# wangrui2025/GDKVM

Hardware: AMD Instinct MI355X
Metric: frames/sec (GDKVM forward + argmax mask), EchoNet 112x112x32 clips (higher is better)
Workload: dtype bf16; 1 GPU; BASELINE.json configs[1]: EchoNet-Dynamic 112x112x32 bf16 inference, batch=16 per GPU; clips_per_gpu=16, frames_per_clip=32, image=112x112, heads=1, key_dim=64, rule=delta_sequential, world_size=1, ranks_seen=1

## Files before the change

gdkvm_amd/csrc/conv3x3_tile.hip:

```cpp
#include <atomic>
#include "gdkvm_device.hpp"

namespace {

constexpr int CT_CK = 64;
constexpr int CT_PIX = 160;
constexpr int CT_SLOTS = CT_PIX / 16;
constexpr int CT_MAXMT = 13;
constexpr int CT_VARIANT_128 = 4, CT_VARIANT_64 = 3;

struct ConvTileArgs {
    const bf16_t* x; const bf16_t* w; const float* bias; const bf16_t* res; bf16_t* y;
    const bf16_t* x2; int C1;
    int N, H, W, C, K;
    int fpt, th, tiles_y, ntiles;
    int bw, bh, band_px, npieces;
    int relu;
    float inv_band, inv_bw, inv_tw, inv_w;
    int perm;
};

__host__ __device__ __forceinline__ int ct_channel(int kt, int j, int perm)
{
    return perm ? 32 * (kt >> 1) + 8 * (j >> 2) + 4 * (kt & 1) + (j & 3) : 16 * kt + j;
}

template <int NWN, int NTW, bool PK, int NWV = 8, int MAXMT = CT_MAXMT>
__global__ __launch_bounds__(64 * NWV, (NWV == 4 ? 2 : 1)) void conv3x3_tile_kernel(ConvTileArgs a)
{
    constexpr int MW = NWV / NWN, MTW = (MAXMT + MW - 1) / MW;
    extern __shared__ __attribute__((aligned(16))) unsigned char ct_band[];
    const int tid = threadIdx.x, lane = tid & 63, li = lane & 15, g = lane >> 4;
    const int w = __builtin_amdgcn_readfirstlane(tid >> 6), wn = w % NWN, wm = w / NWN;
    const int H = a.H, W = a.W, C = a.C, K = a.K, BW = a.bw;
    const int band_bytes = a.npieces * 1024, nchunk = C / CT_CK;
    const int tpix = a.fpt * a.th * W;
    const int co0 = blockIdx.y * (16 * NTW * NWN) + 16 * NTW * wn;

    f32x4 bias4[NTW];
#pragma unroll
    for (int nt = 0; nt < NTW; ++nt) {
        const int kt = min(co0 / 16 + nt, K / 16 - 1);
        const float* bp = a.bias + ct_channel(kt, 4 * g, a.perm);
        asm volatile("global_load_dwordx4 %0, %1, off" : "=&v"(bias4[nt]) : "v"(bp) : "memory");
    }

    constexpr int PP = NWV == 8 ? 7 : 8;
    const int cs1 = a.C1, cs2 = a.x2 ? C - a.C1 : C;
    unsigned g_off1[PP], g_off2[PP];
#pragma unroll
    for (int u = 0; u < PP; ++u) {
        const int j = w + NWV * u, d = 64 * j + lane, pix = d / CT_SLOTS, c = d - CT_SLOTS * pix;
        const int f = idx_div(pix, a.inv_band), r = pix - f * (a.bh * BW), by = idx_div(r, a.inv_bw), bx = r - by * BW;
        const int sp = (f * H + by - 1) * W + bx - 1;
        const bool live = j < a.npieces && c < 8 && pix < a.band_px && bx >= 1 && bx <= W && (a.tiles_y > 1 || (by >= 1 && by <= a.th));
        g_off1[u] = live ? (unsigned)(sp * cs1 * 2 + c * 16) : RSRC_DEAD;
        g_off2[u] = live ? (unsigned)(sp * cs2 * 2 + c * 16) : RSRC_DEAD;
    }
    const unsigned lds0 = (unsigned)reinterpret_cast<uintptr_t>(ct_band);
    const int nlive = max(0, (a.npieces - w + NWV - 1) / NWV);
    struct Geo { int px0, npx, row0; };
    auto geo_of = [&](int tile) __attribute__((always_inline)) {
        const int ty = tile % a.tiles_y, fg = tile / a.tiles_y;
        Geo q;
        q.px0 = fg * a.fpt * H * W;
        q.npx = min(a.fpt, a.N - fg * a.fpt) * H * W;
        q.row0 = ty * a.th * W;
        return q;
    };
    auto fetch = [&](const Geo q, int chunk, int buf) __attribute__((always_inline)) {
        const bool second = a.x2 != nullptr && chunk * CT_CK >= a.C1;
        const int cs = second ? cs2 : cs1;
        const bf16_t* base = (second ? a.x2 : a.x) + (long long)q.px0 * cs;
        const __amdgpu_buffer_rsrc_t rsrc = make_rsrc(base, q.npx * cs * 2);
        const unsigned ts = (unsigned)((q.row0 * cs + chunk * CT_CK - (second ? a.C1 : 0)) * 2);
        const unsigned dst0 = lds0 + buf * band_bytes + 1024 * w;
#pragma unroll
        for (int u = 0; u < PP; ++u) {
            const unsigned dst = u < nlive ? dst0 + 1024 * NWV * u : lds0 + 2 * band_bytes;
            __builtin_amdgcn_raw_ptr_buffer_load_lds(rsrc, lds_dma_dst(dst), 16,
                                                     (int)((second ? g_off2[u] : g_off1[u]) + ts), 0, 0, 0);
        }
    };

    int tile = blockIdx.x;
    Geo cur = geo_of(min(tile, a.ntiles - 1));
    if (tile < a.ntiles) fetch(cur, 0, 0);

    unsigned pbase[MTW];
#pragma unroll
    for (int m = 0; m < MTW; ++m) {
        const int p = min(16 * (wm + MW * m) + li, tpix - 1);
        const int f = idx_div(p, a.inv_tw), r = p - f * (a.th * W), py = idx_div(r, a.inv_w), px = r - py * W;
        pbase[m] = (unsigned)(((f * a.bh + py) * BW + px) * CT_PIX + g * 16);
    }
    const bf16_t* wrow[NTW];
#pragma unroll
    for (int nt = 0; nt < NTW; ++nt) {
        const int kt = min(co0 / 16 + nt, K / 16 - 1);
        if constexpr (PK) wrow[nt] = a.w + (size_t)kt * (9 * C * 16) + lane * 8;
        else wrow[nt] = a.w + (size_t)ct_channel(kt, li, a.perm) * 9 * C + 8 * g;
    }

    const int nks = nchunk * 18;
    static_assert(NTW == 1 || NTW == 2, "wwait names the fragments of one or two output tiles");
    struct WF { bf16x8 f[NTW]; };
    auto wload = [&](WF& o, int ks) __attribute__((always_inline)) {
        ks = ks >= nks ? ks - nks : ks;
        size_t off;
        if constexpr (PK) off = (size_t)ks * 512;
        else {
            const int chunk = ks / 18, r = ks - 18 * chunk, tap = r >> 1, kh = r & 1;
            off = (size_t)tap * C + chunk * CT_CK + 32 * kh;
        }
#pragma unroll
        for (int nt = 0; nt < NTW; ++nt) asm volatile("global_load_dwordx4 %0, %1, off" : "=&v"(o.f[nt]) : "v"(wrow[nt] + off) : "memory");
    };
    auto wwait = [&](WF& o, auto nc) __attribute__((always_inline)) {
        constexpr int N = decltype(nc)::value;
        if constexpr (NTW == 1) asm volatile("s_waitcnt vmcnt(%1)" : "+v"(o.f[0]) : "n"(N) : "memory");
        else asm volatile("s_waitcnt vmcnt(%2)" : "+v"(o.f[0]), "+v"(o.f[1]) : "n"(N) : "memory");
    };
    int gc = 0;
    constexpr int WD = 3, KU = 6;
    WF wr[WD];
#pragma unroll
    for (int j = 0; j < WD; ++j) wload(wr[j], j);
    for (; tile < a.ntiles; tile += gridDim.x) {
        const Geo nxt = geo_of(min(tile + (int)gridDim.x, a.ntiles - 1));
        f32x4 acc[MTW][NTW];
#pragma unroll
        for (int m = 0; m < MTW; ++m)
#pragma unroll
            for (int nt = 0; nt < NTW; ++nt) acc[m][nt] = f32x4{0.f, 0.f, 0.f, 0.f};
        for (int chunk = 0; chunk < nchunk; ++chunk, ++gc) {
            const int buf = gc & 1;
            asm volatile("s_waitcnt vmcnt(%0) lgkmcnt(0)" ::"n"(WD * NTW) : "memory");
            asm volatile("s_barrier" ::: "memory");
            {
                const bool more = chunk + 1 < nchunk;
                Geo q;
                q.px0 = more ? cur.px0 : nxt.px0; q.npx = more ? cur.npx : nxt.npx; q.row0 = more ? cur.row0 : nxt.row0;
                fetch(q, more ? chunk + 1 : 0, buf ^ 1);
            }
            const unsigned char* band = ct_band + buf * band_bytes;
            auto load_x = [&](bf16x8 (&xb)[MTW], int r) __attribute__((always_inline)) {
                r = min(r, 17);
                const int tap = r >> 1, kh = r & 1, dy = tap / 3, dx = tap - 3 * dy;
                const unsigned off = (unsigned)((dy * BW + dx) * CT_PIX + kh * 64);
#pragma unroll
                for (int m = 0; m < MTW; ++m) {
                    xb[m] = *reinterpret_cast<const bf16x8*>(band + pbase[m] + off);
                }
            };
            auto mfmas = [&](const bf16x8 (&xb)[MTW], const WF& wfr) __attribute__((always_inline)) {
#pragma unroll
                for (int m = 0; m < MTW; ++m)
#pragma unroll
                    for (int nt = 0; nt < NTW; ++nt) {
                        acc[m][nt] = __builtin_amdgcn_mfma_f32_16x16x32_bf16(wfr.f[nt], xb[m], acc[m][nt], 0, 0, 0);
                    }
            };
            const int ksb = chunk * 18;
            bf16x8 xa[MTW], xb[MTW];
            load_x(xa, 0);
            auto trip = [&](int r0, auto firstc) __attribute__((always_inline)) {
                constexpr bool FIRST = decltype(firstc)::value;
                static_for<0, KU>([&](auto jc) {
                    constexpr int j = decltype(jc)::value;
                    wwait(wr[j % WD], std::integral_constant<int, (WD - 1) * NTW + (FIRST && j < WD ? PP : 0)>{});
                    if constexpr (j % 2 == 0) { load_x(xb, r0 + j + 1); mfmas(xa, wr[j % WD]); }
                    else { load_x(xa, r0 + j + 1); mfmas(xb, wr[j % WD]); }
                    wload(wr[j % WD], ksb + r0 + j + WD);
                    __builtin_amdgcn_sched_barrier(0);
                });
            };
            trip(0, std::true_type{});
#pragma unroll 1
            for (int r0 = KU; r0 < 18; r0 += KU) trip(r0, std::false_type{});
        }
        {
            const int ty = tile % a.tiles_y, fg = tile / a.tiles_y;
            const float lo = a.relu ? 0.f : -INFINITY;
            if (NTW == 2 && a.perm) {
                if (co0 < K) {
                    unsigned o[MTW];
#pragma unroll
                    for (int m = 0; m < MTW; ++m) {
                        const int p = 16 * (wm + MW * m) + li;
                        const int pc = min(p, tpix - 1);
                        const int f = idx_div(pc, a.inv_tw), r = pc - f * (a.th * W), py = idx_div(r, a.inv_w), px = r - py * W;
                        const int n = fg * a.fpt + f, yy = ty * a.th + py;
                        o[m] = p < tpix && n < a.N && yy < H ? (unsigned)(((n * H + yy) * W + px) * K + co0 + 8 * g) : ~0u;
                    }
                    bf16_t* const yout = a.y;
                    const bf16_t* const resp = a.res;
                    const unsigned ofallback = (unsigned)(co0 + 8 * g);
                    auto finish = [&](auto resc) __attribute__((always_inline)) {
                        constexpr bool RES = decltype(resc)::value;
                        static_for<0, (MTW + 3) / 4>([&](auto bc) {
                            constexpr int M0 = 4 * decltype(bc)::value, M1 = M0 + 4 < MTW ? M0 + 4 : MTW;
                            u32x4 rr[4] = {};
                            if constexpr (RES) {
#pragma unroll
                                for (int m = M0; m < M1; ++m)
                                {
                                    const bf16_t* const rp = resp + (o[m] != ~0u ? o[m] : ofallback);
                                    asm volatile("global_load_dwordx4 %0, %1, off" : "=&v"(rr[m - M0]) : "v"(rp) : "memory");
                                }
                                asm volatile("s_waitcnt vmcnt(0)" : "+v"(rr[0]), "+v"(rr[1]), "+v"(rr[2]), "+v"(rr[3]) :: "memory");
                            }
#pragma unroll
                            for (int m = M0; m < M1; ++m) {
                                f32x2 v[4];
#pragma unroll
                                for (int q = 0; q < 4; ++q)
                                    v[q] = f32x2{acc[m][q >> 1][2 * (q & 1)], acc[m][q >> 1][2 * (q & 1) + 1]} + f32x2{bias4[q >> 1][2 * (q & 1)], bias4[q >> 1][2 * (q & 1) + 1]};
                                if constexpr (RES) {
#pragma unroll
                                    for (int q = 0; q < 4; ++q) v[q] += unpack_bf16x2(rr[m - M0][q]);
                                }
                                u32x4 ow;
#pragma unroll
                                for (int q = 0; q < 4; ++q) {
                                    v[q] = __builtin_elementwise_max(v[q], f32x2{lo, lo});
                                    ow[q] = pack_bf16x2(v[q][0], v[q][1]);
                                }
                                bf16_t* const yp = yout + o[m];
                                if (o[m] != ~0u) asm volatile("global_store_dwordx4 %0, %1, off\n\ts_nop 1" :: "v"(yp), "v"(ow) : "memory");
                            }
                        });
                    };
                    if (a.res) finish(std::true_type{}); else finish(std::false_type{});
                }
            } else {
#pragma unroll
                for (int m = 0; m < MTW; ++m) {
                    const int p = 16 * (wm + MW * m) + li;
                    if (p >= tpix) continue;
                    const int f = idx_div(p, a.inv_tw), r = p - f * (a.th * W), py = idx_div(r, a.inv_w), px = r - py * W;
                    const int n = fg * a.fpt + f, yy = ty * a.th + py;
                    if (n >= a.N || yy >= H) continue;
                    const size_t opix = (((size_t)n * H + yy) * W + px) * K;
#pragma unroll
                    for (int nt = 0; nt < NTW; ++nt) {
                        if (co0 + 16 * nt >= K) continue;
                        const size_t o = opix + ct_channel(co0 / 16 + nt, 4 * g, a.perm);
                        f32x4 v = acc[m][nt] + bias4[nt];
                        if (a.res) v += unpack_bf16x4(*reinterpret_cast<const uint2*>(a.res + o));
                        v = __builtin_elementwise_max(v, f32x4{lo, lo, lo, lo});
                        *reinterpret_cast<uint2*>(a.y + o) = pack_bf16x4(v);
                    }
                }
            }
        }
        cur = nxt;
    }
    asm volatile("s_waitcnt vmcnt(0)" ::: "memory");
}

__global__ __launch_bounds__(256) void conv3x3_pack_kernel(const uint4* w, uint4* packed, int K, int C)
{
    const int nks = C / CT_CK * 18;
    const size_t total = (size_t)(K / 16) * nks * 64;
    for (size_t i = (size_t)blockIdx.x * 256 + threadIdx.x; i < total; i += (size_t)gridDim.x * 256) {
        const int lane = (int)(i & 63), li = lane & 15, g = lane >> 4;
        const size_t f = i >> 6;
        const int ks = (int)(f % nks), kt = (int)(f / nks);
        const int chunk = ks / 18, r = ks - 18 * chunk, tap = r >> 1, kh = r & 1;
        packed[i] = w[(((size_t)ct_channel(kt, li, K % 32 == 0) * 9 + tap) * C + chunk * CT_CK + 32 * kh + 8 * g) / 8];
    }
}

__global__ __launch_bounds__(256) void conv3x3_pack_dgrad_kernel(const bf16_t* w, uint4* packed, int K, int C)
{
    const int nks = K / CT_CK * 18;
    const size_t total = (size_t)(C / 16) * nks * 64;
    for (size_t i = (size_t)blockIdx.x * 256 + threadIdx.x; i < total; i += (size_t)gridDim.x * 256) {
        const int lane = (int)(i & 63), li = lane & 15, g = lane >> 4;
        const size_t f = i >> 6;
        const int ks = (int)(f % nks), ct = (int)(f / nks);
        const int chunk = ks / 18, r = ks - 18 * chunk, tap = r >> 1, kh = r & 1;
        const int c = ct_channel(ct, li, C % 32 == 0), ftap = 8 - tap;
        const bf16_t* src = w + ((size_t)(chunk * CT_CK + 32 * kh + 8 * g) * 9 + ftap) * C + c;
        unsigned short e[8];
#pragma unroll
        for (int j = 0; j < 8; ++j) e[j] = src[(size_t)j * 9 * C];
        packed[i] = make_uint4(e[0] | (unsigned)e[1] << 16, e[2] | (unsigned)e[3] << 16, e[4] | (unsigned)e[5] << 16, e[6] | (unsigned)e[7] << 16);
    }
}

}

struct PackTrainLayer { const float* w; uint4* fwd; uint4* dgrad; int K, C; long long sK, sC, sR, sS; };
struct PackTrainArgs { PackTrainLayer l[GDKVM_PACK_MAX_LAYERS]; };

namespace {
__global__ __launch_bounds__(256) void conv3x3_pack_train_kernel(PackTrainArgs a)
{
    const PackTrainLayer L = a.l[blockIdx.y];
    if (!L.w) return;
    const int K = L.K, C = L.C;
    const size_t nf = (size_t)(K / 16) * (C / CT_CK * 18) * 64, nd = (size_t)(C / 16) * (K / CT_CK * 18) * 64;
    for (size_t i = (size_t)blockIdx.x * 256 + threadIdx.x; i < nf + nd; i += (size_t)gridDim.x * 256) {
        const bool fwd = i < nf;
        const size_t ii = fwd ? i : i - nf;
        const int lane = (int)(ii & 63), li = lane & 15, g = lane >> 4;
        const size_t f = ii >> 6;
        float e[8];
        if (fwd) {
            const int nks = C / CT_CK * 18, ks = (int)(f % nks), kt = (int)(f / nks);
            const int chunk = ks / 18, r = ks - 18 * chunk, tap = r >> 1, kh = r & 1;
            const float* src = L.w + (long long)ct_channel(kt, li, K % 32 == 0) * L.sK + (long long)(tap / 3) * L.sR + (long long)(tap % 3) * L.sS
                               + (long long)(chunk * CT_CK + 32 * kh + 8 * g) * L.sC;
#pragma unroll
            for (int j = 0; j < 8; ++j) e[j] = src[(long long)j * L.sC];
        } else {
            const int nks = K / CT_CK * 18, ks = (int)(f % nks), ct = (int)(f / nks);
            const int chunk = ks / 18, r = ks - 18 * chunk, tap = r >> 1, kh = r & 1, ftap = 8 - tap;
            const float* src = L.w + (long long)ct_channel(ct, li, C % 32 == 0) * L.sC + (long long)(ftap / 3) * L.sR + (long long)(ftap % 3) * L.sS
                               + (long long)(chunk * CT_CK + 32 * kh + 8 * g) * L.sK;
#pragma unroll
            for (int j = 0; j < 8; ++j) e[j] = src[(long long)j * L.sK];
        }
        const uint4 o = pack_bf16x8(e);
        (fwd ? L.fwd : L.dgrad)[ii] = o;
    }
}
}

extern "C" int gdkvm_conv3x3_pack_weights_train(int nlayers, const void* const* w, void* const* packed_fwd, void* const* packed_dgrad,
                                                const int* K, const int* C, const long long* strides, void* stream)
{
    if (nlayers < 0 || nlayers > GDKVM_PACK_MAX_LAYERS) return gdkvm_fail(GDKVM_ERR_SHAPE, "conv3x3_pack_weights_train: %d layers (at most %d per call)", nlayers, GDKVM_PACK_MAX_LAYERS);
    if (nlayers == 0) return GDKVM_OK;
    if (!w || !packed_fwd || !packed_dgrad || !K || !C || !strides) return gdkvm_fail(GDKVM_ERR_ARG, "conv3x3_pack_weights_train: null pointer");
    PackTrainArgs a{};
    for (int i = 0; i < nlayers; ++i) {
        if (K[i] <= 0 || C[i] <= 0 || K[i] % CT_CK || C[i] % CT_CK)
            return gdkvm_fail(GDKVM_ERR_SHAPE, "conv3x3_pack_weights_train: layer %d K=%d C=%d (multiples of 64)", i, K[i], C[i]);
        if (!w[i] || !packed_fwd[i] || !packed_dgrad[i] || !gdkvm_aligned16(packed_fwd[i]) || !gdkvm_aligned16(packed_dgrad[i]))
            return gdkvm_fail(GDKVM_ERR_ARG, "conv3x3_pack_weights_train: layer %d: null or unaligned pointer", i);
        a.l[i] = PackTrainLayer{static_cast<const float*>(w[i]), static_cast<uint4*>(packed_fwd[i]), static_cast<uint4*>(packed_dgrad[i]), K[i], C[i],
                                strides[4 * i], strides[4 * i + 1], strides[4 * i + 2], strides[4 * i + 3]};
    }
    if (int rc = gdkvm_check_device()) return rc;
    hipLaunchKernelGGL(conv3x3_pack_train_kernel, dim3(48, (unsigned)nlayers), dim3(256), 0, static_cast<hipStream_t>(stream), a);
    GDKVM_LAUNCH_CHECK("conv3x3_pack_train_kernel");
    return GDKVM_OK;
}

extern "C" int gdkvm_conv3x3_pack_weights_dgrad(const void* w, void* packed, int K, int C, int io_dtype, void* stream)
{
    if (io_dtype != GDKVM_BF16) return gdkvm_fail(GDKVM_ERR_DTYPE, "conv3x3_pack_weights_dgrad: only bf16 is implemented");
    if (K <= 0 || C <= 0 || K % CT_CK || C % 16) return gdkvm_fail(GDKVM_ERR_SHAPE, "conv3x3_pack_weights_dgrad: K=%d C=%d (K a multiple of 64, C of 16)", K, C);
    if (!w || !packed || !gdkvm_aligned16(w) || !gdkvm_aligned16(packed)) return gdkvm_fail(GDKVM_ERR_ARG, "conv3x3_pack_weights_dgrad: null or unaligned pointer");
    if (int rc = gdkvm_check_device()) return rc;
    const size_t total = (size_t)(C / 16) * (K / CT_CK * 18) * 64;
    hipLaunchKernelGGL(conv3x3_pack_dgrad_kernel, dim3((unsigned)((total + 255) / 256)), dim3(256), 0, static_cast<hipStream_t>(stream),
                       static_cast<const bf16_t*>(w), static_cast<uint4*>(packed), K, C);
    GDKVM_LAUNCH_CHECK("conv3x3_pack_dgrad_kernel");
    return GDKVM_OK;
}

extern "C" int gdkvm_conv3x3_pack_weights(const void* w, void* packed, int K, int C, int io_dtype, void* stream)
{
    if (io_dtype != GDKVM_BF16) return gdkvm_fail(GDKVM_ERR_DTYPE, "conv3x3_pack_weights: only bf16 is implemented");
    if (K <= 0 || C <= 0 || K % 16 || C % CT_CK) return gdkvm_fail(GDKVM_ERR_SHAPE, "conv3x3_pack_weights: K=%d C=%d (K a multiple of 16, C of 64)", K, C);
    if (!w || !packed || !gdkvm_aligned16(w) || !gdkvm_aligned16(packed)) return gdkvm_fail(GDKVM_ERR_ARG, "conv3x3_pack_weights: null or unaligned pointer");
    if (int rc = gdkvm_check_device()) return rc;
    const size_t total = (size_t)(K / 16) * (C / CT_CK * 18) * 64;
    hipLaunchKernelGGL(conv3x3_pack_kernel, dim3((unsigned)((total + 255) / 256)), dim3(256), 0, static_cast<hipStream_t>(stream),
                       static_cast<const uint4*>(w), static_cast<uint4*>(packed), K, C);
    GDKVM_LAUNCH_CHECK("conv3x3_pack_kernel");
    return GDKVM_OK;
}

namespace {
template <int NWN, int NTW, int NWV = 8, int MAXMT = CT_MAXMT>
void launch_tile(bool packed, dim3 grid, size_t lds, hipStream_t st, const ConvTileArgs& a)
{
    if (packed) hipLaunchKernelGGL((conv3x3_tile_kernel<NWN, NTW, true, NWV, MAXMT>), grid, dim3(64 * NWV), lds, st, a);
    else hipLaunchKernelGGL((conv3x3_tile_kernel<NWN, NTW, false, NWV, MAXMT>), grid, dim3(64 * NWV), lds, st, a);
}
template <int NWN, int NTW, int NWV = 8, int MAXMT = CT_MAXMT>
bool setattr_tile()
{
    return hipFuncSetAttribute(reinterpret_cast<const void*>(conv3x3_tile_kernel<NWN, NTW, true, NWV, MAXMT>), hipFuncAttributeMaxDynamicSharedMemorySize, 113 * 1024) == hipSuccess
        && hipFuncSetAttribute(reinterpret_cast<const void*>(conv3x3_tile_kernel<NWN, NTW, false, NWV, MAXMT>), hipFuncAttributeMaxDynamicSharedMemorySize, 113 * 1024) == hipSuccess;
}
}

int gdkvm_conv3x3_tile_launch(const void* x, const void* x2, int C1, const void* w, const float* bias, const void* residual, void* y,
                              int N, int C, int H, int W, int K, int relu, int variant, int packed, hipStream_t st)
{
    if (variant == 0 && K % 128 == 0 && CT_VARIANT_128 == 4) {
        if (gdkvm_conv3x3_tile_launch(x, x2, C1, w, bias, residual, y, N, C, H, W, K, relu, 4, packed, st) == 0) return 0;
        variant = 2;
    }
    if (variant == 0 && K % 128 != 0 && (H * W <= 16 * 7 || 2 * W <= 16 * 7)) {
        if (gdkvm_conv3x3_tile_launch(x, x2, C1, w, bias, residual, y, N, C, H, W, K, relu, 5, packed, st) == 0) return 0;
        variant = 3;
    }
    if (C % CT_CK || K % 16 || W > 64 || W < 1 || H < 1 || N < 1 || variant < 0 || variant > 5) return 1;
    if (variant == 4 && K % 128) return 1;
    const bool half = variant == 4 || variant == 5;
    if (x2 && (C1 <= 0 || C1 >= C || C1 % CT_CK)) return 1;
    ConvTileArgs a;
    a.x2 = static_cast<const bf16_t*>(x2); a.C1 = x2 ? C1 : C;
    a.x = static_cast<const bf16_t*>(x); a.w = static_cast<const bf16_t*>(w); a.bias = bias;
    a.res = static_cast<const bf16_t*>(residual); a.y = static_cast<bf16_t*>(y);
    a.N = N; a.H = H; a.W = W; a.C = C; a.K = K; a.relu = relu;
    const int maxpix = half ? 16 * 7 : 16 * CT_MAXMT;
    const int maxpieces = half ? 32 : 56;
    if (H * W <= maxpix) { a.th = H; a.fpt = maxpix / (H * W); a.tiles_y = 1; if (a.fpt > N) a.fpt = N; }
    else { a.fpt = 1; a.th = maxpix / W; if (a.th < 1) return 1; a.tiles_y = (H + a.th - 1) / a.th; }
    a.bw = W + 2; a.bh = a.th + 2;
    auto pieces = [&]() { a.band_px = a.fpt * a.bh * a.bw; return (a.band_px * CT_SLOTS + 63) / 64; };
    while (pieces() > maxpieces && a.fpt > 1) --a.fpt;
    while (pieces() > maxpieces && a.th > 1) { --a.th; a.bh = a.th + 2; a.tiles_y = (H + a.th - 1) / a.th; }
    a.npieces = pieces();
    if (a.npieces > maxpieces) return 1;
    if ((long long)(a.fpt * H + 2) * W * (x2 ? (C1 > C - C1 ? C1 : C - C1) : C) * 2 >= 0x7fffffffLL) return 1;
    a.inv_band = 1.0f / (float)(a.bh * a.bw); a.inv_bw = 1.0f / (float)a.bw;
    a.inv_tw = 1.0f / (float)(a.th * W); a.inv_w = 1.0f / (float)W;
    a.perm = K % 32 == 0;
    const long long groups = (N + a.fpt - 1) / a.fpt;
    const long long ntiles = groups * a.tiles_y;
    if (ntiles <= 0 || ntiles > 0x7fffffffLL) return 1;
    a.ntiles = (int)ntiles;
    if (variant == 0) variant = K % 128 == 0 ? 2 : CT_VARIANT_64;
    const int kwg = (variant == 2 || variant == 4) ? 128 : 64;
    const int gy = (K + kwg - 1) / kwg;
    const size_t lds = (size_t)2 * a.npieces * 1024 + 1024;
    int per = (half ? 512 : 256) / gy; if (per < 1) per = 1;
    const int gx = (int)(ntiles < per ? ntiles : per);
    static std::atomic<unsigned long long> done_mask{0};
    int dev = 0;
    if (hipGetDevice(&dev) != hipSuccess) return 1;
    const unsigned long long bit = 1ull << (dev & 63);
    if (!(done_mask.load(std::memory_order_relaxed) & bit)) {
        if (!setattr_tile<4, 1>() || !setattr_tile<4, 2>() || !setattr_tile<2, 2>() || !setattr_tile<4, 2, 4, 7>() || !setattr_tile<2, 2, 4, 7>()) return 1;
        done_mask.fetch_or(bit, std::memory_order_relaxed);
    }
    switch (variant) {
        case 1: launch_tile<4, 1>(packed, dim3(gx, gy), lds, st, a); break;
        case 2: launch_tile<4, 2>(packed, dim3(gx, gy), lds, st, a); break;
        case 4: launch_tile<4, 2, 4, 7>(packed, dim3(gx, gy), lds, st, a); break;
        case 5: launch_tile<2, 2, 4, 7>(packed, dim3(gx, gy), lds, st, a); break;
        default: launch_tile<2, 2>(packed, dim3(gx, gy), lds, st, a); break;
    }
    return 0;
}
```

gdkvm_amd/csrc/conv_igemm.hip:

```cpp
#include <atomic>

#include "gdkvm_device.hpp"

namespace {

constexpr int IG_TN = 128;
constexpr int IG_WAVES_N = 4;
constexpr int IG_GD = 2;

struct IgArgs {
    const bf16_t* x; const bf16_t* w; const float* bias; const bf16_t* res; bf16_t* y;
    int N, H, W, C, K, R, S, stride, pad, Ho, Wo, relu;
    int M, ksteps, cps;
    const bf16_t* w2; const float* bias2; bf16_t* y2; int centre;
    float inv_cps, inv_s;
    struct Cls { const bf16_t* w; int S, ksteps_main, ksteps_all, ksteps_row; float inv_s; } cls[4];
    const bf16_t* x2; int OH, OW;
};

template <int TM, int SUB, int TN = IG_TN, int WN = IG_WAVES_N, bool DG = false>
__global__ __launch_bounds__(256, 2) void conv_igemm_kernel(IgArgs a)
{
    constexpr int NTW = TN / 16 / WN;
    constexpr int MT = TM / 16 / (4 / WN);
    constexpr int PITCH = SUB == 2 ? 160 : 80;
    constexpr int PPP = 4 * SUB;
    constexpr int GP = TM * PPP / 256;
    constexpr int WD = SUB == 2 ? 2 : 3;
    constexpr int UF = SUB == 2 ? 2 : 6;
    __shared__ __attribute__((aligned(16))) unsigned char s_a[2][TM * PITCH];
    const int tid = threadIdx.x, lane = tid & 63, li = lane & 15, g = lane >> 4;
    const int w = __builtin_amdgcn_readfirstlane(tid >> 6), wm = w / WN, wn = w % WN;
    const int m0 = blockIdx.x * TM, n0 = blockIdx.y * TN;
    const int cls = DG ? (int)blockIdx.z : 0;
    const int S_ = DG ? a.cls[cls].S : a.S;
    const float inv_s_ = DG ? a.cls[cls].inv_s : a.inv_s;
    const int nsteps = (DG ? a.cls[cls].ksteps_all : a.ksteps) / SUB;
    const int main_steps = DG ? a.cls[cls].ksteps_main / SUB : nsteps;
    const ptrdiff_t x2_diff = DG && a.x2 ? a.x2 - a.x : 0;

    int g_iy0[GP], g_ix0[GP];
    const bf16_t* g_base[GP];
    unsigned g_lds[GP];
#pragma unroll
    for (int u = 0; u < GP; ++u) {
        const int q = 256 * u + tid, px = q / PPP, part = q % PPP;
        const int gp = min(m0 + px, a.M - 1);
        const int gn = gp / (a.Ho * a.Wo), grem = gp - gn * a.Ho * a.Wo, gyo = grem / a.Wo, gxo = grem - gyo * a.Wo;
        g_iy0[u] = m0 + px < a.M ? gyo * a.stride - a.pad : -0x40000000;
        g_ix0[u] = gxo * a.stride - a.pad;
        g_base[u] = a.x + (size_t)gn * a.H * a.W * a.C + 8 * part;
        g_lds[u] = (unsigned)(px * PITCH + 16 * part);
    }
    uint4 ga[IG_GD][GP];
    unsigned gok[IG_GD];
    const int spt = a.cps / SUB;
    const float inv_spt = a.inv_cps * (float)SUB;
    auto gather = [&](int st, uint4 (&d)[GP], unsigned& okm) __attribute__((always_inline)) {
        const bool second = DG && st >= main_steps;
        const int stm = second ? st - main_steps : st;
        const int tap = idx_div(stm, inv_spt), c0 = (stm - tap * spt) * 32 * SUB, r = idx_div(tap, inv_s_), s = tap - r * S_;
        const ptrdiff_t src = second ? x2_diff : 0;
        okm = 0;
#pragma unroll
        for (int u = 0; u < GP; ++u) {
            const int iy = g_iy0[u] + r, ix = g_ix0[u] + s;
            const bool ok = (unsigned)iy < (unsigned)a.H && (unsigned)ix < (unsigned)a.W;
            okm |= ok ? 1u << u : 0u;
            d[u] = *reinterpret_cast<const uint4*>(g_base[u] + src + ((size_t)(ok ? iy : 0) * a.W + (ok ? ix : 0)) * a.C + c0);
        }
    };
    auto put = [&](int buf, const uint4 (&d)[GP], unsigned okm) __attribute__((always_inline)) {
#pragma unroll
        for (int u = 0; u < GP; ++u) {
            const unsigned m = (okm >> u) & 1u ? 0xffffffffu : 0u;
            *reinterpret_cast<uint4*>(&s_a[buf][g_lds[u]]) = make_uint4(d[u].x & m, d[u].y & m, d[u].z & m, d[u].w & m);
        }
    };

    const unsigned abase = (unsigned)((16 * MT * wm + li) * PITCH + 16 * g);

    auto run_pass = [&](const bf16_t* wpk, int g0, int L, const float* bias, const bf16_t* res, bf16_t* y, int relu, int Lrow) __attribute__((always_inline)) {
        const bf16_t* wp = wpk + ((size_t)((n0 + 16 * NTW * wn) / 16) * (Lrow * SUB) * 64 + lane) * 8;
        const size_t nt_stride = (size_t)(Lrow * SUB) * 512;
        bf16x8 wr[WD][SUB][NTW];
        auto wload = [&](int l, bf16x8 (&d)[SUB][NTW]) __attribute__((always_inline)) {
            const size_t off = (size_t)min(l, L - 1) * (512 * SUB);
#pragma unroll
            for (int sb = 0; sb < SUB; ++sb)
#pragma unroll
                for (int nt = 0; nt < NTW; ++nt) d[sb][nt] = *reinterpret_cast<const bf16x8*>(wp + nt * nt_stride + off + 512 * sb);
        };
        const int glast = g0 + L - 1;
        f32x4 acc[MT][NTW];
#pragma unroll
        for (int mt = 0; mt < MT; ++mt)
#pragma unroll
            for (int nt = 0; nt < NTW; ++nt) acc[mt][nt] = f32x4{0.f, 0.f, 0.f, 0.f};

        gather(min(g0, glast), ga[0], gok[0]);
        gather(min(g0 + 1, glast), ga[1], gok[1]);
#pragma unroll
        for (int d = 0; d < WD; ++d) wload(d, wr[d]);
        put(0, ga[0], gok[0]);
        gather(min(g0 + 2, glast), ga[0], gok[0]);
        __syncthreads();

        auto step = [&](int l, auto jc) __attribute__((always_inline)) {
            constexpr int j = decltype(jc)::value % WD, gs = (decltype(jc)::value + 1) & 1;
            const int buf = l & 1;
#pragma unroll
            for (int sb = 0; sb < SUB; ++sb)
#pragma unroll
                for (int mt = 0; mt < MT; ++mt) {
                    const bf16x8 xa = *reinterpret_cast<const bf16x8*>(&s_a[buf][abase + mt * 16 * PITCH + 64 * sb]);
#pragma unroll
                    for (int nt = 0; nt < NTW; ++nt) acc[mt][nt] = __builtin_amdgcn_mfma_f32_16x16x32_bf16(wr[j][sb][nt], xa, acc[mt][nt], 0, 0, 0);
                }
            put(buf ^ 1, ga[gs], gok[gs]);
            wload(l + WD, wr[j]);
            gather(min(g0 + l + 1 + IG_GD, glast), ga[gs], gok[gs]);
            __syncthreads();
        };
        int l = 0;
        for (; l + UF <= L; l += UF)
            static_for<0, UF>([&](auto jc) { step(l + decltype(jc)::value, jc); });
        static_for<0, UF - 1>([&](auto jc) { if (l + decltype(jc)::value < L) step(l + decltype(jc)::value, jc); });

        const float lo = relu ? 0.f : -INFINITY;
#pragma unroll
        for (int nt = 0; nt < NTW; ++nt) {
            const int ch = n0 + 16 * NTW * wn + 16 * nt + 4 * g;
            const f32x4 b4 = bias ? *reinterpret_cast<const f32x4*>(bias + ch) : f32x4{0.f, 0.f, 0.f, 0.f};
#pragma unroll
            for (int mt = 0; mt < MT; ++mt) {
                const int p = m0 + 16 * MT * wm + 16 * mt + li;
                if (p >= a.M) continue;
                f32x4 v = acc[mt][nt] + b4;
                size_t o = (size_t)p * a.K + ch;
                if constexpr (DG) {
                    const int pn = p / (a.Ho * a.Wo), prem = p - pn * a.Ho * a.Wo, ya = prem / a.Wo, xb = prem - ya * a.Wo;
                    const int oy = 2 * ya + (cls >> 1), ox = 2 * xb + (cls & 1);
                    if (oy >= a.OH || ox >= a.OW) continue;
                    o = (((size_t)pn * a.OH + oy) * a.OW + ox) * a.K + ch;
                }
                if (res) {
                    const uint2 rr = *reinterpret_cast<const uint2*>(res + o);
                    v[0] += bf16_lo(rr.x); v[1] += bf16_hi(rr.x);
                    v[2] += bf16_lo(rr.y); v[3] += bf16_hi(rr.y);
                }
#pragma unroll
                for (int r = 0; r < 4; ++r) v[r] = fmaxf(v[r], lo);
                *reinterpret_cast<uint2*>(y + o) = make_uint2(pack_bf16x2(v[0], v[1]), pack_bf16x2(v[2], v[3]));
            }
        }
    };
    if constexpr (DG) {
        run_pass(a.cls[cls].w, 0, nsteps, nullptr, nullptr, a.y, 0, a.cls[cls].ksteps_row / SUB);
    } else {
        run_pass(a.w, 0, nsteps, a.bias, a.res, a.y, a.relu, nsteps);
        if (a.w2) run_pass(a.w2, a.centre * spt, spt, a.bias2, nullptr, a.y2, 0, spt);
    }
}

__global__ __launch_bounds__(256) void conv_igemm_pack_kernel(const uint4* w, uint4* packed, int K, int Kd)
{
    const int nks = Kd / 32;
    const size_t total = (size_t)(K / 16) * nks * 64;
    for (size_t i = (size_t)blockIdx.x * 256 + threadIdx.x; i < total; i += (size_t)gridDim.x * 256) {
        const int lane = (int)(i & 63), li = lane & 15, g = lane >> 4;
        const size_t f = i >> 6;
        const int ks = (int)(f % nks), nt = (int)(f / nks);
        packed[i] = w[((size_t)(16 * nt + li) * Kd + 32 * ks + 8 * g) / 8];
    }
}

}

extern "C" int gdkvm_conv_igemm_pack_weights(const void* w, void* packed, int K, int C, int R, int S, int io_dtype, void* stream)
{
    if (io_dtype != GDKVM_BF16) return gdkvm_fail(GDKVM_ERR_DTYPE, "conv_igemm_pack_weights: only bf16 is implemented");
    if (K <= 0 || C <= 0 || R <= 0 || S <= 0 || K % 16 || C % 32)
        return gdkvm_fail(GDKVM_ERR_SHAPE, "conv_igemm_pack_weights: K=%d C=%d %dx%d (K a multiple of 16, C of 32)", K, C, R, S);
    if (!w || !packed || !gdkvm_aligned16(w) || !gdkvm_aligned16(packed)) return gdkvm_fail(GDKVM_ERR_ARG, "conv_igemm_pack_weights: null or unaligned pointer");
    if (int rc = gdkvm_check_device()) return rc;
    const int Kd = R * S * C;
    const size_t total = (size_t)(K / 16) * (Kd / 32) * 64;
    hipLaunchKernelGGL(conv_igemm_pack_kernel, dim3((unsigned)((total + 255) / 256 > 4096 ? 4096 : (total + 255) / 256)), dim3(256), 0,
                       static_cast<hipStream_t>(stream), static_cast<const uint4*>(w), static_cast<uint4*>(packed), K, Kd);
    GDKVM_LAUNCH_CHECK("conv_igemm_pack_kernel");
    return GDKVM_OK;
}

int gdkvm_conv_igemm_launch(const void* x, const void* wpacked, const float* bias, const void* residual, void* y,
                            int N, int C, int H, int W, int K, int R, int S, int stride, int pad, int relu,
                            const void* w2packed, const float* bias2, void* y2, hipStream_t st)
{
    if (C % 32 || K % IG_TN || N < 1 || R < 1 || S < 1 || stride < 1 || pad < 0) return 1;
    if (w2packed && (!y2 || R != S || !(R & 1) || pad != R / 2)) return 1;
    const int Ho = (H + 2 * pad - R) / stride + 1, Wo = (W + 2 * pad - S) / stride + 1;
    if (Ho < 1 || Wo < 1) return 1;
    const long long M = (long long)N * Ho * Wo;
    if (M * (long long)(K > C ? K : C) > 0x7fffffffLL || (long long)N * H * W * C > 0x7fffffffLL || (long long)R * S * C / 32 > 65535) return 1;
    IgArgs a{};
    a.x = static_cast<const bf16_t*>(x); a.w = static_cast<const bf16_t*>(wpacked); a.bias = bias;
    a.res = static_cast<const bf16_t*>(residual); a.y = static_cast<bf16_t*>(y);
    a.w2 = static_cast<const bf16_t*>(w2packed); a.bias2 = bias2; a.y2 = static_cast<bf16_t*>(y2); a.centre = (R / 2) * S + S / 2;
    a.N = N; a.H = H; a.W = W; a.C = C; a.K = K; a.R = R; a.S = S; a.stride = stride; a.pad = pad; a.Ho = Ho; a.Wo = Wo; a.relu = relu;
    a.M = (int)M; a.cps = C / 32; a.ksteps = R * S * a.cps;
    a.inv_cps = 1.0f / (float)a.cps; a.inv_s = 1.0f / (float)S;
    const dim3 grid((unsigned)((M + 127) / 128), (unsigned)(K / IG_TN));
    if (C % 64 == 0) hipLaunchKernelGGL((conv_igemm_kernel<128, 2>), grid, dim3(256), 0, st, a);
    else hipLaunchKernelGGL((conv_igemm_kernel<128, 1>), grid, dim3(256), 0, st, a);
    return 0;
}

int gdkvm_conv_igemm_dgrad_launch(const void* dy, const void* dy2, const void* packs, int with_down, void* dx, int N, int Cf, int H, int W, int Kf, hipStream_t st)
{
    if (Cf % 64 || Kf % 64 || N < 1 || H < 1 || W < 1) return 1;
    const int Ho = (H - 1) / 2 + 1, Wo = (W - 1) / 2 + 1;
    const long long M = (long long)N * Ho * Wo;
    if (M * Kf > 0x7fffffffLL || (long long)N * H * W * Cf > 0x7fffffffLL || 5LL * Kf / 32 > 65535) return 1;
    IgArgs a{};
    a.x = static_cast<const bf16_t*>(dy); a.x2 = static_cast<const bf16_t*>(dy2); a.y = static_cast<bf16_t*>(dx);
    a.N = N; a.H = Ho; a.W = Wo; a.C = Kf; a.K = Cf; a.R = 1; a.S = 1; a.stride = 1; a.pad = 0; a.Ho = Ho; a.Wo = Wo; a.relu = 0;
    a.OH = H; a.OW = W;
    a.M = (int)M; a.cps = Kf / 32; a.ksteps = a.cps;
    a.inv_cps = 1.0f / (float)a.cps; a.inv_s = 1.0f;
    const bf16_t* wp = static_cast<const bf16_t*>(packs);
    for (int c = 0; c < 4; ++c) {
        const int ph = c >> 1, pw = c & 1, taps = (1 + ph) * (1 + pw);
        a.cls[c].w = wp;
        a.cls[c].S = 1 + pw;
        a.cls[c].inv_s = 1.0f / (float)(1 + pw);
        a.cls[c].ksteps_main = taps * a.cps;
        a.cls[c].ksteps_all = (taps + (c == 0 && dy2 && with_down ? 1 : 0)) * a.cps;
        a.cls[c].ksteps_row = (taps + (c == 0 && with_down ? 1 : 0)) * a.cps;
        wp += gdkvm_conv_s2_dgrad_pack_elems(Cf, Kf, c, with_down);
    }
    if (Cf % 128 == 0) {
        const dim3 grid((unsigned)((M + 127) / 128), (unsigned)(Cf / 128), 4);
        hipLaunchKernelGGL((conv_igemm_kernel<128, 2, 128, 4, true>), grid, dim3(256), 0, st, a);
    } else {
        const dim3 grid((unsigned)((M + 127) / 128), (unsigned)(Cf / 64), 4);
        hipLaunchKernelGGL((conv_igemm_kernel<128, 2, 64, 2, true>), grid, dim3(256), 0, st, a);
    }
    return 0;
}
```

Before: 642,200 frames/s.

## Use buffer loads with explicit vmcnt pipelining in conv epilogue and igemm mainloop

The conv3x3 tile epilogue switches from global loads and stores with per-group full waits to buffer_load/store through a resource descriptor. Out-of-range pixels are handled by a dead offset that the hardware bounds check drops, and the code waits per row with a partial vmcnt. In the non-DG igemm path, the activation gather uses buffer loads whose per-thread base offsets are computed once, replacing per-tap address and mask computation. The main loop is rescheduled with hand-placed vmcnt/lgkmcnt waits, double-buffered LDS fragment reads and sched barriers so loads overlap the MFMA work. This adds a 32-bit offset limit check and relies on fragile inline asm counter bookkeeping.

```diff
diff --git a/gdkvm_amd/csrc/conv3x3_tile.hip b/gdkvm_amd/csrc/conv3x3_tile.hip
--- a/gdkvm_amd/csrc/conv3x3_tile.hip
+++ b/gdkvm_amd/csrc/conv3x3_tile.hip
@@ -184,52 +184,50 @@
             const float lo = a.relu ? 0.f : -INFINITY;
             if (NTW == 2 && a.perm) {
                 if (co0 < K) {
+                    const unsigned ts = (unsigned)(cur.row0 * K * 2), fbytes = (unsigned)(cur.npx * K * 2);
                     unsigned o[MTW];
 #pragma unroll
                     for (int m = 0; m < MTW; ++m) {
                         const int p = 16 * (wm + MW * m) + li;
                         const int pc = min(p, tpix - 1);
                         const int f = idx_div(pc, a.inv_tw), r = pc - f * (a.th * W), py = idx_div(r, a.inv_w), px = r - py * W;
-                        const int n = fg * a.fpt + f, yy = ty * a.th + py;
-                        o[m] = p < tpix && n < a.N && yy < H ? (unsigned)(((n * H + yy) * W + px) * K + co0 + 8 * g) : ~0u;
+                        o[m] = (p < tpix ? (unsigned)((((f * H + py) * W + px) * K + co0 + 8 * g) * 2) : RSRC_DEAD) + ts;
                     }
-                    bf16_t* const yout = a.y;
-                    const bf16_t* const resp = a.res;
-                    const unsigned ofallback = (unsigned)(co0 + 8 * g);
+                    const unsigned long long ya = reinterpret_cast<unsigned long long>(a.y + (long long)cur.px0 * K);
+                    const unsigned long long ra = reinterpret_cast<unsigned long long>(a.res + (long long)cur.px0 * K);
+                    const u32x4 yrs = {(unsigned)ya, (unsigned)(ya >> 32) & 0xffffu, fbytes, (unsigned)RSRC_WORD3};
+                    const u32x4 rrs = {(unsigned)ra, (unsigned)(ra >> 32) & 0xffffu, fbytes, (unsigned)RSRC_WORD3};
                     auto finish = [&](auto resc) __attribute__((always_inline)) {
                         constexpr bool RES = decltype(resc)::value;
-                        static_for<0, (MTW + 3) / 4>([&](auto bc) {
-                            constexpr int M0 = 4 * decltype(bc)::value, M1 = M0 + 4 < MTW ? M0 + 4 : MTW;
-                            u32x4 rr[4] = {};
+                        u32x4 rr[MTW] = {};
+                        const u32x4 rs = rrs, ys = yrs;
+                        if constexpr (RES) {
+#pragma unroll
+                            for (int m = 0; m < MTW; ++m) {
+                                const unsigned om = o[m];
+                                asm volatile("buffer_load_dwordx4 %0, %1, %2, 0 offen" : "=&v"(rr[m]) : "v"(om), "s"(rs) : "memory");
+                            }
+                        }
+#pragma unroll
+                        for (int m = 0; m < MTW; ++m) {
+                            f32x2 v[4];
+#pragma unroll
+                            for (int q = 0; q < 4; ++q)
+                                v[q] = f32x2{acc[m][q >> 1][2 * (q & 1)], acc[m][q >> 1][2 * (q & 1) + 1]} + f32x2{bias4[q >> 1][2 * (q & 1)], bias4[q >> 1][2 * (q & 1) + 1]};
                             if constexpr (RES) {
-#pragma unroll
-                                for (int m = M0; m < M1; ++m)
-                                {
-                                    const bf16_t* const rp = resp + (o[m] != ~0u ? o[m] : ofallback);
-                                    asm volatile("global_load_dwordx4 %0, %1, off" : "=&v"(rr[m - M0]) : "v"(rp) : "memory");
-                                }
-                                asm volatile("s_waitcnt vmcnt(0)" : "+v"(rr[0]), "+v"(rr[1]), "+v"(rr[2]), "+v"(rr[3]) :: "memory");
+                                asm volatile("s_waitcnt vmcnt(%1)" : "+v"(rr[m]) : "n"(MTW - 1) : "memory");
+#pragma unroll
+                                for (int q = 0; q < 4; ++q) v[q] += unpack_bf16x2(rr[m][q]);
                             }
-#pragma unroll
-                            for (int m = M0; m < M1; ++m) {
-                                f32x2 v[4];
-#pragma unroll
-                                for (int q = 0; q < 4; ++q)
-                                    v[q] = f32x2{acc[m][q >> 1][2 * (q & 1)], acc[m][q >> 1][2 * (q & 1) + 1]} + f32x2{bias4[q >> 1][2 * (q & 1)], bias4[q >> 1][2 * (q & 1) + 1]};
-                                if constexpr (RES) {
-#pragma unroll
-                                    for (int q = 0; q < 4; ++q) v[q] += unpack_bf16x2(rr[m - M0][q]);
-                                }
-                                u32x4 ow;
-#pragma unroll
-                                for (int q = 0; q < 4; ++q) {
-                                    v[q] = __builtin_elementwise_max(v[q], f32x2{lo, lo});
-                                    ow[q] = pack_bf16x2(v[q][0], v[q][1]);
-                                }
-                                bf16_t* const yp = yout + o[m];
-                                if (o[m] != ~0u) asm volatile("global_store_dwordx4 %0, %1, off\n\ts_nop 1" :: "v"(yp), "v"(ow) : "memory");
+                            u32x4 ow;
+#pragma unroll
+                            for (int q = 0; q < 4; ++q) {
+                                v[q] = __builtin_elementwise_max(v[q], f32x2{lo, lo});
+                                ow[q] = pack_bf16x2(v[q][0], v[q][1]);
                             }
-                        });
+                            const unsigned om = o[m];
+                            asm volatile("buffer_store_dwordx4 %0, %1, %2, 0 offen\n\ts_nop 1" :: "v"(ow), "v"(om), "s"(ys) : "memory");
+                        }
                     };
                     if (a.res) finish(std::true_type{}); else finish(std::false_type{});
                 }
@@ -422,6 +420,7 @@
     a.npieces = pieces();
     if (a.npieces > maxpieces) return 1;
     if ((long long)(a.fpt * H + 2) * W * (x2 ? (C1 > C - C1 ? C1 : C - C1) : C) * 2 >= 0x7fffffffLL) return 1;
+    if ((long long)(a.fpt * H + a.th) * W * K * 2 >= 0x7fffffffLL) return 1;
     a.inv_band = 1.0f / (float)(a.bh * a.bw); a.inv_bw = 1.0f / (float)a.bw;
     a.inv_tw = 1.0f / (float)(a.th * W); a.inv_w = 1.0f / (float)W;
     a.perm = K % 32 == 0;
diff --git a/gdkvm_amd/csrc/conv_igemm.hip b/gdkvm_amd/csrc/conv_igemm.hip
--- a/gdkvm_amd/csrc/conv_igemm.hip
+++ b/gdkvm_amd/csrc/conv_igemm.hip
@@ -7,6 +7,7 @@
 constexpr int IG_TN = 128;
 constexpr int IG_WAVES_N = 4;
 constexpr int IG_GD = 2;
+constexpr unsigned IG_DEAD = 0xffffffe0u;
 
 struct IgArgs {
     const bf16_t* x; const bf16_t* w; const float* bias; const bf16_t* res; bf16_t* y;
@@ -78,6 +79,35 @@
         }
     };
 
+    unsigned g_off0[GP];
+    u32x4 xrs = {};
+    if constexpr (!DG) {
+#pragma unroll
+        for (int u = 0; u < GP; ++u) {
+            const int q = 256 * u + tid, px = q / PPP, part = q % PPP;
+            const int gp = min(m0 + px, a.M - 1);
+            const int gn = gp / (a.Ho * a.Wo);
+            g_off0[u] = ((((unsigned)gn * a.H + (unsigned)g_iy0[u]) * a.W + (unsigned)g_ix0[u]) * a.C + 8 * part) * 2;
+        }
+        const unsigned long long xa = reinterpret_cast<unsigned long long>(a.x);
+        xrs = u32x4{(unsigned)xa, (unsigned)(xa >> 32) & 0xffffu, (unsigned)a.N * a.H * a.W * a.C * 2, (unsigned)RSRC_WORD3};
+    }
+    auto gather_d = [&](int st, u32x4 (&d)[GP]) __attribute__((always_inline)) {
+        const int tap = idx_div(st, inv_spt), c0 = (st - tap * spt) * 32 * SUB, r = idx_div(tap, inv_s_), s = tap - r * S_;
+        const unsigned srel = (unsigned)(((r * a.W + s) * a.C + c0) * 2);
+#pragma unroll
+        for (int u = 0; u < GP; ++u) {
+            const bool ok = (unsigned)(g_iy0[u] + r) < (unsigned)a.H && (unsigned)(g_ix0[u] + s) < (unsigned)a.W;
+            const unsigned off = ok ? g_off0[u] + srel : IG_DEAD;
+            asm volatile("buffer_load_dwordx4 %0, %1, %2, 0 offen" : "=&v"(d[u]) : "v"(off), "s"(xrs) : "memory");
+        }
+    };
+    auto put_d = [&](int buf, const u32x4 (&d)[GP]) __attribute__((always_inline)) {
+#pragma unroll
+        for (int u = 0; u < GP; ++u) *reinterpret_cast<u32x4*>(&s_a[buf][g_lds[u]]) = d[u];
+    };
+    u32x4 gd[IG_GD][GP];
+
     const unsigned abase = (unsigned)((16 * MT * wm + li) * PITCH + 16 * g);
 
     auto run_pass = [&](const bf16_t* wpk, int g0, int L, const float* bias, const bf16_t* res, bf16_t* y, int relu, int Lrow) __attribute__((always_inline)) {
@@ -98,34 +128,110 @@
 #pragma unroll
             for (int nt = 0; nt < NTW; ++nt) acc[mt][nt] = f32x4{0.f, 0.f, 0.f, 0.f};
 
-        gather(min(g0, glast), ga[0], gok[0]);
-        gather(min(g0 + 1, glast), ga[1], gok[1]);
-#pragma unroll
-        for (int d = 0; d < WD; ++d) wload(d, wr[d]);
-        put(0, ga[0], gok[0]);
-        gather(min(g0 + 2, glast), ga[0], gok[0]);
-        __syncthreads();
-
-        auto step = [&](int l, auto jc) __attribute__((always_inline)) {
-            constexpr int j = decltype(jc)::value % WD, gs = (decltype(jc)::value + 1) & 1;
-            const int buf = l & 1;
-#pragma unroll
-            for (int sb = 0; sb < SUB; ++sb)
-#pragma unroll
-                for (int mt = 0; mt < MT; ++mt) {
-                    const bf16x8 xa = *reinterpret_cast<const bf16x8*>(&s_a[buf][abase + mt * 16 * PITCH + 64 * sb]);
-#pragma unroll
-                    for (int nt = 0; nt < NTW; ++nt) acc[mt][nt] = __builtin_amdgcn_mfma_f32_16x16x32_bf16(wr[j][sb][nt], xa, acc[mt][nt], 0, 0, 0);
-                }
-            put(buf ^ 1, ga[gs], gok[gs]);
-            wload(l + WD, wr[j]);
-            gather(min(g0 + l + 1 + IG_GD, glast), ga[gs], gok[gs]);
+        if constexpr (DG) {
+            gather(min(g0, glast), ga[0], gok[0]);
+            gather(min(g0 + 1, glast), ga[1], gok[1]);
+#pragma unroll
+            for (int d = 0; d < WD; ++d) wload(d, wr[d]);
+            put(0, ga[0], gok[0]);
+            gather(min(g0 + 2, glast), ga[0], gok[0]);
             __syncthreads();
-        };
-        int l = 0;
-        for (; l + UF <= L; l += UF)
-            static_for<0, UF>([&](auto jc) { step(l + decltype(jc)::value, jc); });
-        static_for<0, UF - 1>([&](auto jc) { if (l + decltype(jc)::value < L) step(l + decltype(jc)::value, jc); });
+
+            auto step = [&](int l, auto jc) __attribute__((always_inline)) {
+                constexpr int j = decltype(jc)::value % WD, gs = (decltype(jc)::value + 1) & 1;
+                const int buf = l & 1;
+#pragma unroll
+                for (int sb = 0; sb < SUB; ++sb)
+#pragma unroll
+                    for (int mt = 0; mt < MT; ++mt) {
+                        const bf16x8 xa = *reinterpret_cast<const bf16x8*>(&s_a[buf][abase + mt * 16 * PITCH + 64 * sb]);
+#pragma unroll
+                        for (int nt = 0; nt < NTW; ++nt) acc[mt][nt] = __builtin_amdgcn_mfma_f32_16x16x32_bf16(wr[j][sb][nt], xa, acc[mt][nt], 0, 0, 0);
+                    }
+                put(buf ^ 1, ga[gs], gok[gs]);
+                wload(l + WD, wr[j]);
+                gather(min(g0 + l + 1 + IG_GD, glast), ga[gs], gok[gs]);
+                __syncthreads();
+            };
+            int l = 0;
+            for (; l + UF <= L; l += UF)
+                static_for<0, UF>([&](auto jc) { step(l + decltype(jc)::value, jc); });
+            static_for<0, UF - 1>([&](auto jc) { if (l + decltype(jc)::value < L) step(l + decltype(jc)::value, jc); });
+        } else {
+            constexpr int WL = SUB * NTW, PS = WL + GP, W_YOUNGER = (WD - 1) * PS, G_YOUNGER = WL + (IG_GD - 1) * PS;
+            static_assert(WL == GP && (GP == 2 || GP == 4), "landed() names the registers of a set of two or four loads");
+            auto landed = [&](auto& r0, auto& r1, auto& r2, auto& r3, auto nc) __attribute__((always_inline)) {
+                constexpr int N = decltype(nc)::value;
+                if constexpr (GP == 2) asm volatile("s_waitcnt vmcnt(%2)" : "+v"(r0), "+v"(r1) : "n"(N) : "memory");
+                else asm volatile("s_waitcnt vmcnt(%4)" : "+v"(r0), "+v"(r1), "+v"(r2), "+v"(r3) : "n"(N) : "memory");
+            };
+            auto wlanded = [&](bf16x8 (&d)[SUB][NTW], auto nc) __attribute__((always_inline)) { landed(d[0][0], d[0][1], d[SUB - 1][0], d[SUB - 1][1], nc); };
+            auto glanded = [&](u32x4 (&d)[GP], auto nc) __attribute__((always_inline)) { landed(d[0], d[1], d[GP - 2], d[GP - 1], nc); };
+            const unsigned wlane = (unsigned)lane * 16;
+            const bf16_t* const wrow = wpk + (size_t)((n0 + 16 * NTW * wn) / 16) * (Lrow * SUB) * 512;
+            auto wload_a = [&](int l, bf16x8 (&d)[SUB][NTW]) __attribute__((always_inline)) {
+                const bf16_t* const ws = wrow + (size_t)min(l, L - 1) * (512 * SUB);
+#pragma unroll
+                for (int sb = 0; sb < SUB; ++sb)
+#pragma unroll
+                    for (int nt = 0; nt < NTW; ++nt)
+                        asm volatile("global_load_dwordx4 %0, %1, %2 offset:%3" : "=&v"(d[sb][nt]) : "v"(wlane), "s"(ws + nt * nt_stride), "n"(1024 * sb) : "memory");
+            };
+            if constexpr (WD == 3) wload_a(0, wr[0]);
+            gather_d(min(g0, glast), gd[0]);
+            gather_d(min(g0 + 1, glast), gd[1]);
+            wload_a(WD - 2, wr[WD - 2]);
+            glanded(gd[0], std::integral_constant<int, PS>{});
+            put_d(0, gd[0]);
+            gather_d(min(g0 + 2, glast), gd[0]);
+            wload_a(WD - 1, wr[WD - 1]);
+            asm volatile("s_waitcnt lgkmcnt(0)\n\ts_barrier" ::: "memory");
+
+            constexpr int FG = 4, NG = SUB * MT / FG;
+            static_assert(SUB * MT % FG == 0 && NG >= 2, "fragment groups");
+            auto step = [&](int l, auto jc) __attribute__((always_inline)) {
+                constexpr int j = decltype(jc)::value % WD, gs = (decltype(jc)::value + 1) & 1;
+                const int buf = l & 1;
+                bf16x8 xf[2][FG];
+                auto read = [&](auto gc) __attribute__((always_inline)) {
+                    constexpr int G = decltype(gc)::value;
+#pragma unroll
+                    for (int i = 0; i < FG; ++i) {
+                        const int f = G * FG + i, sb = f / MT, mt = f % MT;
+                        xf[G & 1][i] = *reinterpret_cast<const bf16x8*>(&s_a[buf][abase + mt * 16 * PITCH + 64 * sb]);
+                    }
+                };
+                wlanded(wr[j], std::integral_constant<int, W_YOUNGER>{});
+                read(std::integral_constant<int, 0>{});
+                static_for<0, NG>([&](auto gc) {
+                    constexpr int G = decltype(gc)::value;
+                    if constexpr (G + 1 < NG) read(std::integral_constant<int, G + 1>{});
+#pragma unroll
+                    for (int i = 0; i < FG; ++i) {
+                        const int f = G * FG + i, sb = f / MT, mt = f % MT;
+#pragma unroll
+                        for (int nt = 0; nt < NTW; ++nt) acc[mt][nt] = __builtin_amdgcn_mfma_f32_16x16x32_bf16(wr[j][sb][nt], xf[G & 1][i], acc[mt][nt], 0, 0, 0);
+                    }
+                    __builtin_amdgcn_sched_barrier(0);
+                    if constexpr (G == NG / 2 - 1) {
+                        glanded(gd[gs], std::integral_constant<int, G_YOUNGER>{});
+                        put_d(buf ^ 1, gd[gs]);
+                        gather_d(min(g0 + l + 1 + IG_GD, glast), gd[gs]);
+                        __builtin_amdgcn_sched_barrier(0);
+                    }
+                });
+                wload_a(l + WD, wr[j]);
+                asm volatile("s_waitcnt lgkmcnt(0)\n\ts_barrier" ::: "memory");
+                __builtin_amdgcn_sched_barrier(0);
+            };
+            int l = 0;
+            for (; l + UF <= L; l += UF)
+                static_for<0, UF>([&](auto jc) { step(l + decltype(jc)::value, jc); });
+            static_for<0, UF - 1>([&](auto jc) { if (l + decltype(jc)::value < L) step(l + decltype(jc)::value, jc); });
+            static_for<0, WD>([&](auto dc) { wlanded(wr[decltype(dc)::value], std::integral_constant<int, 0>{}); });
+            glanded(gd[0], std::integral_constant<int, 0>{});
+            glanded(gd[1], std::integral_constant<int, 0>{});
+        }
 
         const float lo = relu ? 0.f : -INFINITY;
 #pragma unroll
```

After: 642,800 frames/s, median of 2. No clear change (+0.1%).
